# DanielLin94144/E2E-ASR-Pytorch

Hardware: AMD Instinct MI355X
Metric: audio frames/sec (fwd+bwd) LibriSpeech-100 joint CTC-att (higher is better)
Workload: dtype bf16; 1 GPU; config/librispeech_asr.yaml (vgg 0, 4xBiLSTM-320, joint CTC-att 0.5), B=16 x T=1200 x D=160 per GPU, L=180, delta+SpecAugment on GPU, fwd+losses+bwd+grad-allreduce+clip+Adadelta, dropout on; global_batch=16, frames_per_utt=1200, parallelism=dp1

## Files before the change

e2e-asr-pytorch_amd/csrc/decoder_cluster.h:

```cpp
#pragma once
#include "common.h"
#include "handoff.h"
#include "decoder_internal.h"
#include <stdlib.h>
#include <algorithm>

namespace {


constexpr u64 PAIR_MASK = 7ull | (7ull << 32);
__device__ __forceinline__ u64 pair_want(unsigned seq, unsigned epoch) {
    epoch = 2u + epoch % 14u;
    const unsigned tag = ((epoch & 15u) << 2) | seq;
    return (u64)(tag & 7u) | ((u64)(tag >> 3) << 32);
}
__device__ __forceinline__ u64 pack2(float a, float b, u64 want) {
    return ((u64)(__float_as_uint(a) & ~7u) | ((u64)(__float_as_uint(b) & ~7u) << 32)) | want;
}
__device__ __forceinline__ float lo_f(u64 g) { return __uint_as_float((unsigned)g & ~7u); }
__device__ __forceinline__ float hi_f(u64 g) { return __uint_as_float((unsigned)(g >> 32) & ~7u); }
__device__ __forceinline__ unsigned f2h_bits(float x) { return (unsigned)__builtin_bit_cast(unsigned short, (_Float16)x); }
__device__ __forceinline__ u64 pack4h(float a, float b, float c, float d, u64 want) {
    const unsigned lo = (f2h_bits(a) & ~7u) | (f2h_bits(b) << 16), hi = (f2h_bits(c) & ~7u) | (f2h_bits(d) << 16);
    return ((u64)lo | ((u64)hi << 32)) | want;
// ... 35 lines not shown
__device__ __forceinline__ float tanh_f(float x) { return 1.f - 2.f * __builtin_amdgcn_rcpf(1.f + __expf(2.f * x)); }
__device__ __forceinline__ float sigm_f(float x) { return __builtin_amdgcn_rcpf(1.f + __expf(-x)); }

__device__ __forceinline__ float wave_sum_dpp(float v) {
#define DPB_STEP(CTRL, RMASK) v += __builtin_bit_cast(float, __builtin_amdgcn_update_dpp(0, __builtin_bit_cast(int, v), CTRL, RMASK, 0xf, false));
    DPB_STEP(0xB1, 0xf)
    DPB_STEP(0x4E, 0xf)
    DPB_STEP(0x141, 0xf)
    DPB_STEP(0x140, 0xf)
    DPB_STEP(0x142, 0xa)
    DPB_STEP(0x143, 0xc)
#undef DPB_STEP
    return __builtin_bit_cast(float, __builtin_amdgcn_readlane(__builtin_bit_cast(int, v), 63));
}
__device__ __forceinline__ float sum8_dpp(float v) {
    v += __builtin_bit_cast(float, __builtin_amdgcn_update_dpp(0, __builtin_bit_cast(int, v), 0xB1, 0xf, 0xf, false));
    v += __builtin_bit_cast(float, __builtin_amdgcn_update_dpp(0, __builtin_bit_cast(int, v), 0x4E, 0xf, 0xf, false));
    v += __builtin_bit_cast(float, __builtin_amdgcn_update_dpp(0, __builtin_bit_cast(int, v), 0x141, 0xf, 0xf, false));
    return v;
}
__device__ __forceinline__ float wave_max_dpp(float v) {
#define DPB_STEP(CTRL, RMASK) v = fmaxf(v, __builtin_bit_cast(float, __builtin_amdgcn_update_dpp(__builtin_bit_cast(int, v), __builtin_bit_cast(int, v), CTRL, RMASK, 0xf, false)));
    DPB_STEP(0xB1, 0xf)
    DPB_STEP(0x4E, 0xf)
    DPB_STEP(0x141, 0xf)
    DPB_STEP(0x140, 0xf)
    DPB_STEP(0x142, 0xa)
    DPB_STEP(0x143, 0xc)
#undef DPB_STEP
    return __builtin_bit_cast(float, __builtin_amdgcn_readlane(__builtin_bit_cast(int, v), 63));
}

struct PD {
    asr_dec_dims_t d;
    asr_dec_weights_t w;
    asr_dec_state_t s;
    const float* enc;
    const int64_t* enc_len;
    const unsigned short* wcat16;
    const float* embproj;
    u64* xbuf;
    unsigned* status;
    int NT, TE, UPW, QPW, CPW;
    int HG2, QG2, SG2;
    int KC, KCP;
    int allow_local;
    unsigned epoch;
};

struct ConvGeo { int NKS, WKP, IMG_LD, need; };
__host__ __device__ inline ConvGeo conv_geo(int TEB, int Ks) {
    ConvGeo g;
    g.NKS = (2 * Ks + 1 + 31) >> 5;
    g.WKP = 32 * g.NKS + 8;
    g.need = ((TEB + 15) & ~15) + 32 * g.NKS + 8;
    g.IMG_LD = ((g.need - 32 + 127) / 128) * 128 + 32;
    return g;
}
__host__ __device__ inline int conv_img_shorts(const ConvGeo& g) { return 8 * g.IMG_LD + 32 * g.WKP; }

struct FCarve { int cvx_shorts, img, shorts, WT, ATP, NG, x2, q, wg, attp, wc, epart, e, w, g, cpart, stage, stage_floats, floats; };
__host__ __device__ inline FCarve fwd_carve(int TEB, int NT, int A, int E, int Kn, int Ks, int KCP, int UPW, int SG2) {
    FCarve c;
    c.cvx_shorts = TEB * FCVX_LD;
    c.img = (c.cvx_shorts + 7) & ~7;
    c.shorts = (c.img + conv_img_shorts(conv_geo(TEB, Ks)) + 7) & ~7;
    c.WT = (2 * Ks + 1 + 3) & ~3;
    c.ATP = (NT * TEB + 2 * Ks + 8 + 3) & ~3;
    const int nch = E >> 3;
    c.NG = (64 * NCW) / nch; if (c.NG > 8) c.NG = 8;
    int o = 0;
    c.x2 = o; o += 2 * KCP;
    c.q = o; o += (A + 3) & ~3;
    c.wg = o; o += (A + 3) & ~3;
    c.attp = o; o += c.ATP;
    c.wc = o;
    c.epart = o; o += NCW * TEB;
    c.e = o; o += TEB;
    c.w = o; o += TEB;
    c.g = o; o += (4 * UPW + 3) & ~3;
    c.cpart = o; o += c.NG * E;
    c.stage = o;
    c.stage_floats = NT * 2 * SG2; if (c.stage_floats < Kn * TEB) c.stage_floats = Kn * TEB;
    o += c.stage_floats;
    c.floats = o;
    return c;
}

__device__ inline void conv_build_wimg(const float* __restrict__ Wconv, int Kn, int taps, const ConvGeo& g, unsigned short* wimg, int tid, int nthr) {
    for (int i = tid; i < 16 * g.WKP; i += nthr) {
        const int n = i / g.WKP, x = i - n * g.WKP;
        const float v = (n < Kn && x < taps) ? Wconv[n * taps + x] : 0.f;
        const __bf16 hi = (__bf16)v, lo = (__bf16)(v - (float)hi);
        wimg[i] = __builtin_bit_cast(unsigned short, hi);
        wimg[16 * g.WKP + i] = __builtin_bit_cast(unsigned short, lo);
    }
}

__device__ inline void conv_build_ximg(const float* src, int navail, const ConvGeo& g, unsigned short* ximg, int tz, int nthr) {
    const int ngrp = g.IMG_LD >> 2;
    for (int it = tz; it < 4 * ngrp; it += nthr) {
        const int c = it / ngrp, gq = it - c * ngrp;
        unsigned short h[4], l[4];
#pragma unroll
        for (int e = 0; e < 4; ++e) {
            const int i = 4 * gq + c + e;
            const float v = (i < navail && i < g.need) ? src[i] : 0.f;
            const __bf16 hi = (__bf16)v, lo = (__bf16)(v - (float)hi);
            h[e] = __builtin_bit_cast(unsigned short, hi); l[e] = __builtin_bit_cast(unsigned short, lo);
        }
        *reinterpret_cast<uint2*>(ximg + (long)c * g.IMG_LD + 4 * gq) = make_uint2((unsigned)h[0] | ((unsigned)h[1] << 16), (unsigned)h[2] | ((unsigned)h[3] << 16));
        *reinterpret_cast<uint2*>(ximg + (long)(4 + c) * g.IMG_LD + 4 * gq) = make_uint2((unsigned)l[0] | ((unsigned)l[1] << 16), (unsigned)l[2] | ((unsigned)l[3] << 16));
    }
}

template <int NW, class Epi>
__device__ inline void conv_mfma(const unsigned short* ximg, const unsigned short* wimg, const ConvGeo& g, int MTB, int wave, int lane, Epi epi) {
    constexpr int CT = 3;
    const int m = lane & 15, q = lane >> 4, cc = m & 3;
    const unsigned short* xh = ximg + (long)cc * g.IMG_LD + (m - cc) + 8 * q;
    const unsigned short* xl = xh + 4 * g.IMG_LD;
    const unsigned short* wh = wimg + m * g.WKP + 8 * q;
    const unsigned short* wl = wh + 16 * g.WKP;
    for (int mt0 = wave; mt0 < MTB; mt0 += NW * CT) {
        f32x4 acc[CT];
#pragma unroll
        for (int c = 0; c < CT; ++c) acc[c] = f32x4{0.f, 0.f, 0.f, 0.f};
        for (int ks = 0; ks < g.NKS; ++ks) {
            const bf16x8 bh = *reinterpret_cast<const bf16x8*>(wh + 32 * ks), bl = *reinterpret_cast<const bf16x8*>(wl + 32 * ks);
#pragma unroll
            for (int c = 0; c < CT; ++c) {
                const int mt = mt0 + NW * c;
                if (mt < MTB) {
                    const unsigned short* ph = xh + 16 * mt + 32 * ks;
                    const unsigned short* pl = xl + 16 * mt + 32 * ks;
                    const uint2 h0 = *reinterpret_cast<const uint2*>(ph), h1 = *reinterpret_cast<const uint2*>(ph + 4);
                    const uint2 l0 = *reinterpret_cast<const uint2*>(pl), l1 = *reinterpret_cast<const uint2*>(pl + 4);
                    const bf16x8 ah = __builtin_bit_cast(bf16x8, make_uint4(h0.x, h0.y, h1.x, h1.y));
                    const bf16x8 al = __builtin_bit_cast(bf16x8, make_uint4(l0.x, l0.y, l1.x, l1.y));
                    acc[c] = mma16(bh, ah, acc[c]);
                    acc[c] = mma16(bl, ah, acc[c]);
                    acc[c] = mma16(bh, al, acc[c]);
                }
            }
        }
#pragma unroll
        for (int c = 0; c < CT; ++c) {
            const int mt = mt0 + NW * c;
            if (mt < MTB) epi(mt, m, q, acc[c]);
        }
    }
}

__device__ __forceinline__ void compute_barrier(unsigned* cnt, unsigned& gen) {
    gen += NCW;
    __builtin_amdgcn_fence(__ATOMIC_RELEASE, "workgroup");
    if ((threadIdx.x & 63) == 0) {
        __hip_atomic_fetch_add(cnt, 1u, __ATOMIC_RELAXED, __HIP_MEMORY_SCOPE_WORKGROUP);
        while (__hip_atomic_load(cnt, __ATOMIC_RELAXED, __HIP_MEMORY_SCOPE_WORKGROUP) < gen) __builtin_amdgcn_s_sleep(1);
    }
    __builtin_amdgcn_fence(__ATOMIC_ACQUIRE, "workgroup");
}

__global__ void build_wcat16_kernel(const float* __restrict__ wih, const float* __restrict__ whh, unsigned short* __restrict__ out,
                                    int rows, int Dd, int E, int KCP) {
    const long total = (long)rows * KCP;
    for (long i = blockIdx.x * (long)blockDim.x + threadIdx.x; i < total; i += (long)gridDim.x * blockDim.x) {
        const int r = (int)(i / KCP), k = (int)(i - (long)r * KCP);
        float v = 0.f;
        if (k < E) v = wih[(long)r * (Dd + E) + Dd + k];
        else if (k < E + Dd) v = whh[(long)r * Dd + (k - E)];
        out[i] = f2bf_bits(v);
    }
}

template <typename K>
bool grid_resident(K kernel, int grid, int block, size_t lds) {
    int per_cu = 0;
    if (hipOccupancyMaxActiveBlocksPerMultiprocessor(&per_cu, kernel, block, lds) != hipSuccess || per_cu < 1) return false;
    int dev = 0, cus = 0;
    if (hipGetDevice(&dev) != hipSuccess || hipDeviceGetAttribute(&cus, hipDeviceAttributeMultiprocessorCount, dev) != hipSuccess) return false;
    return grid <= cus;
}

template <int CH>
__device__ __forceinline__ void poll_copy(const u64* src, int n16, float* dst, int gt, int np, u64 want, unsigned* status) {
    for (int i0 = gt; i0 < n16; i0 += CH * np) {
        u64 lo[CH], hi[CH];
        int cnt = 0;
#pragma unroll
        for (int k = 0; k < CH; ++k) if (i0 + k * np < n16) cnt = k + 1;
        gather16<CH>(src + 2 * i0, 2 * np, cnt, PAIR_MASK, want, lo, hi, status);
#pragma unroll
        for (int k = 0; k < CH; ++k)
            if (k < cnt) *reinterpret_cast<float4*>(dst + 4 * (long)(i0 + k * np)) = make_float4(lo_f(lo[k]), hi_f(lo[k]), lo_f(hi[k]), hi_f(hi[k]));
    }
}

constexpr int EPOCH_WORD = 1008;
constexpr size_t STATUS_CLEAR_BYTES = 4032;
__global__ void bump_epoch_kernel(unsigned* status) { status[EPOCH_WORD] = status[EPOCH_WORD] + 1u; }
__global__ void clear_work_kernel(uint4* work, long n16) {
    for (long i = blockIdx.x * (long)blockDim.x + threadIdx.x; i < n16; i += (long)gridDim.x * blockDim.x)
        if (i < (long)(STATUS_CLEAR_BYTES / 16) || i >= 256) work[i] = make_uint4(0u, 0u, 0u, 0u);
}
inline void clear_work(void* work, size_t xbuf_bytes, hipStream_t st) {
    const long n16 = (long)((4096 + xbuf_bytes) / 16);
    hipLaunchKernelGGL(clear_work_kernel, dim3((unsigned)std::min<long>((n16 + 255) / 256, 2048)), dim3(256), 0, st, (uint4*)work, n16);
}

}
```

e2e-asr-pytorch_amd/csrc/decoder_persist.hip:

```cpp
#include "decoder_plan.h"

static int g_persist_fwd = -1, g_persist_bwd = -1;
static int g_stream_fwd = -1, g_stream_bwd = -1;
extern "C" int asr_att_decoder_set_persistent(int flags) {
    const int old = (g_persist_fwd != 0 ? 1 : 0) | (g_persist_bwd != 0 ? 2 : 0) | (g_stream_fwd > 0 ? 4 : 0) | (g_stream_bwd > 0 ? 8 : 0);
    g_persist_fwd = flags & 1; g_persist_bwd = (flags >> 1) & 1; g_stream_fwd = (flags >> 2) & 1; g_stream_bwd = (flags >> 3) & 1;
    return old;
}
static void read_switches() {
    if (g_persist_fwd < 0) g_persist_fwd = env_switch("ASR_DEC_PERSIST", 1);
    if (g_persist_bwd < 0) g_persist_bwd = env_switch("ASR_DEC_PERSIST_BWD", 1);
    if (g_stream_fwd < 0) g_stream_fwd = env_switch("ASR_DEC_STREAM", 0);
    if (g_stream_bwd < 0) g_stream_bwd = env_switch("ASR_DEC_STREAM", 0);
}
static FwdPlan fwd_plan(const asr_dec_dims_t& d) { read_switches(); return chosen_plan(persist_plan(d), stream_plan_f(d), g_stream_fwd); }
static BwdPlan bwd_plan(const asr_dec_dims_t& d) { read_switches(); return chosen_plan(persist_plan_b(d), stream_plan_b(d), g_stream_bwd); }

DecPlanInfo dec_fwd_plan_info(const asr_dec_dims_t& d) {
    read_switches();
    const FwdPlan r = persist_plan(d), s = stream_plan_f(d);
    return {chosen_plan(r, s, g_stream_fwd).kind, 0, 0, std::max(r.total, s.total)};
}
DecPlanInfo dec_bwd_plan_info(const asr_dec_dims_t& d) {
    read_switches();
    const BwdPlan r = persist_plan_b(d), s = stream_plan_b(d), pl = chosen_plan(r, s, g_stream_bwd);
    return {pl.kind, pl.NT, std::max(r.NT, s.NT), std::max(r.total, s.total)};
}
float* dec_bwd_dgates(const asr_dec_dims_t& d, void* work) { return bwd_work(d, bwd_plan(d), work).dgates; }

namespace {

size_t dec_fwd_persist_lds(int TE, int NT, int A, int E, int Ks, int KCP, int UPW, int SG2) {
    const int EPL = 16 * cdiv(TE, 16);
    const ConvGeo cg = conv_geo(EPL, Ks);
    const size_t shorts = (size_t)((TE * A + 7) & ~7)
                        + ((TE * E + 7) & ~7)
                        + EPL * FCVX_LD
                        + 8 * cg.IMG_LD
                        + 32 * cg.WKP;
    const size_t floats = (size_t)2 * KCP
                        + ((A + 3) & ~3)
                        + ((A + 3) & ~3)
                        + ((NT * TE + 2 * Ks + 8 + 3) & ~3)
                        + NCW * EPL
                        + ((4 * UPW + 3) & ~3)
                        + (size_t)NT * 2 * SG2;
    return 2 * shorts + 4 * floats;
}

template <int KNMAX, int TPW>
__global__ __launch_bounds__(64 * (NCW + NPW)) void dec_fwd_persist(PD p) {
    constexpr int TE = 8 * TPW;
    constexpr int MT = (TE + 15) / 16;
    constexpr int EPL = 16 * MT;
    extern __shared__ __attribute__((aligned(16))) unsigned char smem[];
    __shared__ unsigned s_bar;
    __shared__ float s_scale[NCW][32];
    const asr_dec_dims_t& d = p.d;
    const int id = blockIdx.x, xcd = id & 7, slot = id >> 3;
    const int cb = slot / p.NT, j = slot - cb * p.NT;
    const int b = cb * 8 + xcd;
    if (b >= d.B) return;
    const unsigned epoch_ = __builtin_amdgcn_readfirstlane(p.status[EPOCH_WORD]);
    const int tid = threadIdx.x, lane = tid & 63, wave = __builtin_amdgcn_readfirstlane(tid >> 6);
    const int NT = p.NT, A = d.A, E = d.E, Dd = d.Dd, Tp = d.Tp, Kn = d.Kn, Ks = d.Ks, L = d.L;
    const int taps = 2 * Ks + 1, XW = Dd + E;
    const int tau0 = j * TE;
    const int len = min((int)p.enc_len[b], Tp);
    const int tmax = max(len - 1, 0);
    unsigned short* s_key = reinterpret_cast<unsigned short*>(smem);
    unsigned short* s_enc = s_key + ((TE * A + 7) & ~7);
    unsigned short* s_cvx = s_enc + ((TE * E + 7) & ~7);
    const ConvGeo cg_ = conv_geo(EPL, Ks);
    unsigned short* s_ximg = s_cvx + EPL * FCVX_LD;
    unsigned short* s_wimg = s_ximg + 8 * cg_.IMG_LD;
    float* s_x2 = reinterpret_cast<float*>(s_wimg + 32 * cg_.WKP);
    float* s_q = s_x2 + 2 * p.KCP;
    float* s_wg = s_q + ((A + 3) & ~3);
    const int WT = (taps + 3) & ~3;
    const int ATP = (NT * TE + 2 * Ks + 8 + 3) & ~3;
    float* s_attp = s_wg + ((A + 3) & ~3);
    float* s_epart = s_attp + ATP;
    float* s_g = s_epart + NCW * EPL;
    float* s_stage = s_g + ((4 * p.UPW + 3) & ~3);
    if (tid == 0) s_bar = 0u;
    const long region = (long)NT * (p.HG2 + p.QG2 + p.SG2);
    auto xb = [&](int parity) { return p.xbuf + ((long)parity * d.B + b) * region; };
    for (int parity = 0; parity < 2; ++parity) {
        u64* base = xb(parity);
        for (int i = tid; i < p.HG2; i += blockDim.x) st_gran_local(base + (long)j * p.HG2 + i, 0ull);
        for (int i = tid; i < p.QG2; i += blockDim.x) st_gran_local(base + (long)NT * p.HG2 + (long)j * p.QG2 + i, 0ull);
        for (int i = tid; i < p.SG2; i += blockDim.x) st_gran_local(base + (long)NT * (p.HG2 + p.QG2) + (long)j * p.SG2 + i, 0ull);
    }
    asm volatile("s_waitcnt vmcnt(0)" ::: "memory");
    __syncthreads();
    const bool local = xcd_consensus(reinterpret_cast<u64*>(p.status) + 64 + b, NT, p.allow_local, p.status);

    for (int i = tid; i < TE * A; i += blockDim.x) {
        const int f = i / A, a = i - f * A;
        s_key[((long)(f >> 2) * A + a) * 4 + (f & 3)] = f2bf_bits(p.s.key[((long)b * Tp + min(tau0 + f, tmax)) * A + a]);
    }
    for (int i = tid; i < TE * E; i += blockDim.x) {
        const int f = i / E, c = i - f * E;
        s_enc[i] = f2bf_bits(p.enc[((long)b * Tp + min(tau0 + f, tmax)) * E + c]);
    }
    for (int i = tid; i < EPL * FCVX_LD; i += blockDim.x) s_cvx[i] = 0;
    conv_build_wimg(p.w.Wconv, Kn, taps, cg_, s_wimg, tid, blockDim.x);
    for (int i = tid; i < A; i += blockDim.x) s_wg[i] = p.w.wg[i];
    for (int i = tid; i < 2 * p.KCP; i += blockDim.x) s_x2[i] = 0.f;
    {
        const float uni = 1.f / (float)max(len, 1);
        for (int i = tid; i < ATP; i += blockDim.x) {
            const int tau = i - Ks;
            s_attp[i] = (tau >= 0 && tau < len) ? uni : 0.f;
        }
    }
    __syncthreads();

    if (wave >= NCW) {
        const int gt = tid - 64 * NCW, np = 64 * NPW;
        for (int t = 0; t < L; ++t) {
            if (t > 0) {
                const u64* src = xb((t - 1) & 1);
                const u64 want = pair_want(seq_of(t - 1), epoch_);
                for (int i0 = gt; 2 * i0 < NT * p.HG2; i0 += np) {
                    u64 lo[1], hi[1];
                    gather16<1>(src + 2 * i0, 0, 1, PAIR_MASK, want, lo, hi, p.status);
                    const int g0 = 2 * i0, prod = g0 / p.HG2, gi = g0 - prod * p.HG2;
                    const int u = prod * p.UPW + 2 * gi;
                    const float v[4] = {lo_f(lo[0]), hi_f(lo[0]), lo_f(hi[0]), hi_f(hi[0])};
#pragma unroll
                    for (int k = 0; k < 4; ++k)
                        if (2 * gi + k < p.UPW && u + k < Dd) s_x2[(t & 1) * p.KCP + E + u + k] = v[k];
                }
            }
            DP_JIT(0)
            __syncthreads();
            DP_JIT(1)
            {
                const u64* src = xb(t & 1) + (long)NT * p.HG2;
                const u64 want = pair_want(seq_of(t), epoch_);
                for (int i0 = gt; 2 * i0 < NT * p.QG2; i0 += np) {
                    u64 lo[1], hi[1];
                    gather16<1>(src + 2 * i0, 0, 1, PAIR_MASK, want, lo, hi, p.status);
                    const int g0 = 2 * i0, prod = g0 / p.QG2, gi = g0 - prod * p.QG2;
                    const int a = prod * p.QPW + 2 * gi;
                    const float v[4] = {lo_f(lo[0]), hi_f(lo[0]), lo_f(hi[0]), hi_f(hi[0])};
#pragma unroll
                    for (int k = 0; k < 4; ++k)
                        if (2 * gi + k < p.QPW && a + k < A) s_q[a + k] = v[k];
                }
            }
            DP_JIT(2)
            __syncthreads();
            DP_JIT(3)
            {
                const u64* src = xb(t & 1) + (long)NT * (p.HG2 + p.QG2);
                const u64 want = pair_want(seq_of(t), epoch_);
                const int npair = NT * p.SG2 / 2;
                for (int i0 = gt; i0 < npair; i0 += 10 * np) {
                    u64 lo[10], hi[10];
                    int cnt = 0;
#pragma unroll
                    for (int k = 0; k < 10; ++k) if (i0 + k * np < npair) cnt = k + 1;
                    gather16<10>(src + 2 * i0, 2 * np, cnt, PAIR_MASK, want, lo, hi, p.status);
#pragma unroll
                    for (int k = 0; k < 10; ++k)
                        if (k < cnt) {
                            float4* o = reinterpret_cast<float4*>(s_stage + 4 * (long)(i0 + k * np));
                            *o = make_float4(lo_f(lo[k]), hi_f(lo[k]), lo_f(hi[k]), hi_f(hi[k]));
                        }
                }
            }
            DP_JIT(4)
            __syncthreads();
            DP_JIT(5)
        }
        return;
    }

    unsigned gen = 0;
    const int u_base = j * p.UPW, q_base = j * p.QPW, c_base = j * p.CPW;
    const int SG2f = 2 * p.SG2;
    const float bg = p.w.bg[0];
    float c_state = 0.f;
    const int RPW = (4 * p.UPW + NCW - 1) / NCW;
    const int nu_cnt = (((A + 15) >> 4) - wave + NCW - 1) / NCW;
    bf16x8 wpx[FSW_NU];
    float wgu[FSW_NU];
    {
        const int q = lane >> 4, c = lane & 15;
#pragma unroll
        for (int nu = 0; nu < FSW_NU; ++nu) {
            const int a = 16 * (wave + NCW * nu) + c;
            const bool ok = a < A;
            const float* wr = p.w.Wproj + (long)min(a, A - 1) * Kn;
#pragma unroll
            for (int i = 0; i < 8; ++i) {
                const int slot = 8 * q + i;
                const int k = slot < KNMAX ? slot : (slot < 2 * KNMAX ? slot - KNMAX : slot - 2 * KNMAX);
                const float w = (ok && slot < 3 * KNMAX && k < Kn) ? wr[min(k, Kn - 1)] : 0.f;
                const __bf16 hi = (__bf16)w;
                wpx[nu][i] = (slot < 2 * KNMAX) ? hi : (__bf16)(w - (float)hi);
            }
            wgu[nu] = ok ? p.w.wg[min(a, A - 1)] : 0.f;
        }
    }
    constexpr int QR = 2;
    float wq0[QR][5], wq1[QR][5], bq0[QR], bq1[QR];
#pragma unroll
    for (int r2 = 0; r2 < QR; ++r2) {
        const int o0 = 2 * wave + 2 * NCW * r2;
        const int a0 = min(q_base + o0, A - 1), a1 = min(q_base + o0 + 1, A - 1);
        bq0[r2] = p.w.bq[a0]; bq1[r2] = p.w.bq[a1];
#pragma unroll
        for (int k = 0; k < 5; ++k) {
            const int kk = min(lane + 64 * k, Dd - 1);
            wq0[r2][k] = p.w.Wq[(long)a0 * Dd + kk];
            wq1[r2][k] = p.w.Wq[(long)a1 * Dd + kk];
        }
    }
    DP_DECL

    for (int t = 0; t < L; ++t) {
        int tz = tid, lz_ = lane;
        asm volatile("" : "+v"(tz), "+v"(lz_));
        const int lane = lz_;
        const long row = (long)b * L + t;
        float* s_x = s_x2 + (t & 1) * p.KCP;
        const u64 want = pair_want(seq_of(t), epoch_);
        u64* out = xb(t & 1);
        float add_r = 0.f;
        {
            const int r = wave * RPW + lane;
            if (lane < RPW && r < 4 * p.UPW) {
                const int g = r / p.UPW, ul = r - g * p.UPW, unit = u_base + ul;
                if (unit < Dd) {
                    const int grow = g * Dd + unit;
                    add_r = p.embproj[row * 4 * Dd + grow] + p.w.bih[0][grow] + p.w.bhh[0][grow];
                }
            }
        }
        DP_MARK(0)
        __syncthreads();
        DP_MARK(1)
        for (int o0 = 2 * wave, rd = 0; o0 < p.QPW; o0 += 2 * NCW, ++rd) {
            float acc0 = 0.f, acc1 = 0.f;
            const int a0 = min(q_base + o0, A - 1), a1 = min(q_base + o0 + 1, A - 1);
            float b0 = 0.f, b1 = 0.f;
            if (rd < QR) {
#pragma unroll
                for (int r2 = 0; r2 < QR; ++r2) if (r2 == rd) { b0 = bq0[r2]; b1 = bq1[r2]; }
            } else {
                b0 = p.w.bq[a0]; b1 = p.w.bq[a1];
            }
            if (t > 0) {
                float w0[5], w1[5];
                if (rd < QR) {
#pragma unroll
                    for (int r2 = 0; r2 < QR; ++r2)
                        if (r2 == rd) {
#pragma unroll
                            for (int k = 0; k < 5; ++k) { w0[k] = wq0[r2][k]; w1[k] = wq1[r2][k]; }
                        }
                } else {
#pragma unroll
                    for (int k = 0; k < 5; ++k) {
                        const int kk = min(lane + 64 * k, Dd - 1);
                        w0[k] = p.w.Wq[(long)a0 * Dd + kk];
                        w1[k] = p.w.Wq[(long)a1 * Dd + kk];
                    }
                }
#pragma unroll
                for (int k = 0; k < 5; ++k) {
                    const float hv = (lane + 64 * k < Dd) ? s_x[E + lane + 64 * k] : 0.f;
                    acc0 += w0[k] * hv; acc1 += w1[k] * hv;
                }
                for (int kk = lane + 320; kk < Dd; kk += 64) { const float hv = s_x[E + kk]; acc0 += p.w.Wq[(long)a0 * Dd + kk] * hv; acc1 += p.w.Wq[(long)a1 * Dd + kk] * hv; }
                acc0 = wave_sum_dpp(acc0); acc1 = wave_sum_dpp(acc1);
            }
            if (lane == 0) {
                const float q0 = tanh_f(acc0 + b0), q1 = tanh_f(acc1 + b1);
                u64* dst = out + (long)NT * p.HG2 + (long)j * p.QG2 + (o0 >> 1);
                if (local) publish<true>(dst, pack2(q0, q1, want)); else publish<false>(dst, pack2(q0, q1, want));
                if (q_base + o0 < A) p.s.q[row * A + q_base + o0] = q0;
                if (o0 + 1 < p.QPW && q_base + o0 + 1 < A) p.s.q[row * A + q_base + o0 + 1] = q1;
            }
        }
        if (tz == 0 && (p.QPW + 1) / 2 < p.QG2) {
            u64* dst = out + (long)NT * p.HG2 + (long)j * p.QG2 + p.QG2 - 1;
            if (local) publish<true>(dst, pack2(0.f, 0.f, want)); else publish<false>(dst, pack2(0.f, 0.f, want));
        }
        DP_MARK(2)
        {
            conv_build_ximg(s_attp + tau0, ATP - tau0, cg_, s_ximg, tz, 64 * NCW);
            compute_barrier(&s_bar, gen);
            conv_mfma<NCW>(s_ximg, s_wimg, cg_, MT, wave, lane, [&](int mt, int n, int q4, const f32x4& acc) {
                const int i = 16 * mt + n;
                unsigned short* r = s_cvx + i * FCVX_LD;
#pragma unroll
                for (int pp = 0; pp < 2; ++pp) {
                    const int k0 = 4 * q4 + 2 * pp;
                    if (k0 < Kn && i < TE) {
                        const float v0 = acc[2 * pp], v1 = acc[2 * pp + 1];
                        const __bf16 h0 = (__bf16)v0, h1 = (__bf16)v1;
                        const __bf16 l0 = (__bf16)(v0 - (float)h0), l1 = (__bf16)(v1 - (float)h1);
                        const unsigned hh = (unsigned)__builtin_bit_cast(unsigned short, h0) | ((unsigned)__builtin_bit_cast(unsigned short, h1) << 16);
                        const unsigned ll = (unsigned)__builtin_bit_cast(unsigned short, l0) | ((unsigned)__builtin_bit_cast(unsigned short, l1) << 16);
                        *reinterpret_cast<unsigned*>(r + k0) = hh;
                        *reinterpret_cast<unsigned*>(r + KNMAX + k0) = ll;
                        *reinterpret_cast<unsigned*>(r + 2 * KNMAX + k0) = hh;
                        if (p.s.conv && tau0 + i < Tp) {
                            p.s.conv[(row * Kn + k0) * Tp + tau0 + i] = v0;
                            if (k0 + 1 < Kn) p.s.conv[(row * Kn + k0 + 1) * Tp + tau0 + i] = v1;
                        }
                    }
                }
            });
        }
        DP_MARK(3)
        __syncthreads();
        DP_MARK(4)
        {
            int opaque = 0;
            asm volatile("" : "+v"(opaque));
            const int q = (lane >> 4) + opaque, c = lane & 15;
            float ep[MT][4];
#pragma unroll
            for (int mt = 0; mt < MT; ++mt)
#pragma unroll
                for (int r = 0; r < 4; ++r) ep[mt][r] = 0.f;
            float qv[FSW_NU];
#pragma unroll
            for (int nu = 0; nu < FSW_NU; ++nu) qv[nu] = s_q[min(16 * (wave + NCW * nu) + c, A - 1)];
#pragma unroll
            for (int mt = 0; mt < MT; ++mt) {
                const int f0 = 16 * mt + 4 * q;
                const bf16x8 av = *reinterpret_cast<const bf16x8*>(s_cvx + (16 * mt + c) * FCVX_LD + 8 * q);
                const int fg = min(f0, TE - 4) >> 2;
#pragma unroll
                for (int nu = 0; nu < FSW_NU; ++nu) {
                    if (nu < nu_cnt) {
                        const int a = min(16 * (wave + NCW * nu) + c, A - 1);
                        const f32x4 lp = mma16(av, wpx[nu], f32x4{0.f, 0.f, 0.f, 0.f});
                        const uint2 kb = *reinterpret_cast<const uint2*>(s_key + ((long)fg * A + a) * 4);
                        const float key[4] = {__uint_as_float(kb.x << 16), __uint_as_float(kb.x & 0xffff0000u),
                                              __uint_as_float(kb.y << 16), __uint_as_float(kb.y & 0xffff0000u)};
#pragma unroll
                        for (int r = 0; r < 4; ++r) ep[mt][r] += wgu[nu] * tanh_f(key[r] + qv[nu] + tanh_f(lp[r]));
                    }
                }
            }
#pragma unroll
            for (int mt = 0; mt < MT; ++mt)
#pragma unroll
                for (int r = 0; r < 4; ++r) {
                    float v = ep[mt][r];
#define DPF_STEP(CTRL) v += __builtin_bit_cast(float, __builtin_amdgcn_update_dpp(0, __builtin_bit_cast(int, v), CTRL, 0xf, 0xf, false));
                    DPF_STEP(0xB1) DPF_STEP(0x4E) DPF_STEP(0x141) DPF_STEP(0x140)
#undef DPF_STEP
                    if (c == 0) s_epart[wave * EPL + 16 * mt + 4 * q + r] = v;
                }
        }
        DP_MARK(5)
        compute_barrier(&s_bar, gen);
        DP_MARK(6)
        {
            float ev = NEG_BIG;
            if (lane < TE) {
                float sv = 0.f;
#pragma unroll
                for (int w8 = 0; w8 < NCW; ++w8) sv += s_epart[w8 * EPL + lane];
                if (tau0 + lane < len) ev = (sv + bg) / d.temperature;
            }
            const float m = wave_max_dpp(ev);
            const float wv = (ev > 0.5f * NEG_BIG) ? __expf(ev - m) : 0.f;
            const float ssum = wave_sum_dpp(wv);
            const int c2 = tz;
            float x0 = 0.f, x1 = 0.f;
            if (2 * c2 < E) {
#pragma unroll
                for (int f = 0; f < TE; ++f) {
                    const float wf = __builtin_bit_cast(float, __builtin_amdgcn_readlane(__builtin_bit_cast(int, wv), f));
                    const unsigned pr = *reinterpret_cast<const unsigned*>(s_enc + f * E + 2 * c2);
                    x0 += wf * __uint_as_float(pr << 16);
                    x1 += wf * __uint_as_float(pr & 0xffff0000u);
                }
            }
            u64* rec = out + (long)NT * (p.HG2 + p.QG2) + (long)j * p.SG2;
            const int ghead = (TE + 2) >> 1;
            const float y0 = __shfl_down(x0, 1), y1 = __shfl_down(x1, 1);
            if (2 * c2 < E && (c2 & 1) == 0) {
                if (local) publish<true>(rec + ghead + (c2 >> 1), pack4h(x0, x1, y0, y1, want)); else publish<false>(rec + ghead + (c2 >> 1), pack4h(x0, x1, y0, y1, want));
            }
            if (wave == NCW - 1) {
                const float e0 = __shfl(ev, min(2 * lane, 63)), e1 = __shfl(ev, min(2 * lane + 1, 63));
                if (lane < TE / 2) {
                    if (local) publish<true>(rec + lane, pack2(e0, e1, want)); else publish<false>(rec + lane, pack2(e0, e1, want));
                } else if (lane == TE / 2) {
                    if (local) publish<true>(rec + lane, pack2(m, ssum, want)); else publish<false>(rec + lane, pack2(m, ssum, want));
                } else if (lane == TE / 2 + 1 && ghead + E / 4 < p.SG2) {
                    u64* dst = rec + p.SG2 - 1;
                    if (local) publish<true>(dst, pack2(0.f, 0.f, want)); else publish<false>(dst, pack2(0.f, 0.f, want));
                }
            }
        }
        DP_MARK(7)
        __syncthreads();
        DP_MARK(8)
        {
            float mi = NEG_BIG, si = 0.f;
            if (lane < NT) { mi = s_stage[lane * SG2f + TE]; si = s_stage[lane * SG2f + TE + 1]; }
            const float M = wave_max_dpp(mi);
            const float wi = (lane < NT) ? si * __expf(mi - M) : 0.f;
            const float S = fmaxf(wave_sum_dpp(wi), 1e-30f);
            const float invS = 1.f / S;
            if (lane < 32) s_scale[wave][lane] = (lane < NT) ? __expf(mi - M) * invS : 0.f;
            __builtin_amdgcn_fence(__ATOMIC_RELEASE, "workgroup");
            __builtin_amdgcn_fence(__ATOMIC_ACQUIRE, "workgroup");
            for (int tau = tz; tau < Tp; tau += 64 * NCW) {
                const int i = tau / TE, f = tau - i * TE;
                const float ev = s_stage[i * SG2f + f];
                const float av = (ev > 0.5f * NEG_BIG) ? __expf(ev - M) * invS : 0.f;
                s_attp[Ks + tau] = av;
                if (i == j) p.s.att[row * Tp + tau] = av;
            }
            for (int c2_ = tz; 2 * c2_ < E; c2_ += 64 * NCW) {
                float a0 = 0.f, a1 = 0.f;
                for (int i = 0; i < NT; ++i) {
                    const unsigned w_ = __float_as_uint(s_stage[i * SG2f + TE + 2 + c2_]);
                    a0 += h2f_lo(w_) * s_scale[wave][i]; a1 += h2f_hi(w_) * s_scale[wave][i];
                }
                const int c = 2 * c2_;
                s_x[c] = a0; s_x[c + 1] = a1;
                if (c >= c_base && c < c_base + p.CPW) p.s.xin[row * XW + Dd + c] = a0;
                if (c + 1 >= c_base && c + 1 < c_base + p.CPW) p.s.xin[row * XW + Dd + c + 1] = a1;
            }
        }
        DP_MARK(9)
        compute_barrier(&s_bar, gen);
        DP_MARK(10)
        {
            constexpr int RBF = 10;
            const int nchunk = p.KCP >> 3;
            float mine = 0.f;
#pragma unroll 1
            for (int bt = 0; bt * RBF < RPW; ++bt) {
                float part[RBF];
#pragma unroll
                for (int rr = 0; rr < RBF; ++rr) part[rr] = 0.f;
                for (int ch0 = lane; ch0 < nchunk; ch0 += 128) {
                    uint4 wv[RBF][2];
#pragma unroll
                    for (int rr = 0; rr < RBF; ++rr) {
                        const int r = min(wave * RPW + bt * RBF + rr, 4 * p.UPW - 1);
                        const int g = r / p.UPW, ul = r - g * p.UPW;
                        const long grow = (long)g * Dd + min(u_base + ul, Dd - 1);
#pragma unroll
                        for (int h2 = 0; h2 < 2; ++h2)
                            wv[rr][h2] = *reinterpret_cast<const uint4*>(p.wcat16 + grow * p.KCP + 8 * min(ch0 + 64 * h2, nchunk - 1));
                    }
#pragma unroll
                    for (int h2 = 0; h2 < 2; ++h2) {
                        const int ch = ch0 + 64 * h2;
                        if (ch < nchunk) {
                            const float4 xa = *reinterpret_cast<const float4*>(s_x + 8 * ch);
                            const float4 xb4 = *reinterpret_cast<const float4*>(s_x + 8 * ch + 4);
#pragma unroll
                            for (int rr = 0; rr < RBF; ++rr) {
                                const uint4 w4 = wv[rr][h2];
                                part[rr] += __uint_as_float(w4.x << 16) * xa.x + __uint_as_float(w4.x & 0xffff0000u) * xa.y +
                                            __uint_as_float(w4.y << 16) * xa.z + __uint_as_float(w4.y & 0xffff0000u) * xa.w +
                                            __uint_as_float(w4.z << 16) * xb4.x + __uint_as_float(w4.z & 0xffff0000u) * xb4.y +
                                            __uint_as_float(w4.w << 16) * xb4.z + __uint_as_float(w4.w & 0xffff0000u) * xb4.w;
                            }
                        }
                    }
                }
#pragma unroll
                for (int rr = 0; rr < RBF; ++rr) {
                    const float sv = wave_sum_dpp(part[rr]);
                    if (lane == bt * RBF + rr) mine = sv;
                }
            }
            const int r = wave * RPW + lane;
            if (lane < RPW && r < 4 * p.UPW) s_g[r] = mine + add_r;
        }
        DP_MARK(11)
        compute_barrier(&s_bar, gen);
        DP_MARK(12)
        if (wave == 0) {
            const int unit = u_base + lane;
            const bool uok = lane < p.UPW && unit < Dd;
            float hv = 0.f;
            float ai = 0.f, af = 0.f, ag = 0.f, ao = 0.f;
            if (uok) {
                ai = sigm_f(s_g[lane]); af = sigm_f(s_g[p.UPW + lane]);
                ag = tanh_f(s_g[2 * p.UPW + lane]); ao = sigm_f(s_g[3 * p.UPW + lane]);
                c_state = af * c_state + ai * ag;
                hv = ao * tanh_f(c_state);
            }
            const float hn = __shfl_down(hv, 1);
            if (t + 1 < L && (lane & 1) == 0 && lane < 2 * p.HG2) {
                u64* dst = out + (long)j * p.HG2 + (lane >> 1);
                if (local) publish<true>(dst, pack2(hv, hn, want)); else publish<false>(dst, pack2(hv, hn, want));
            }
            if (uok) {
                float* go = p.s.gates + row * 4 * Dd;
                go[unit] = ai; go[Dd + unit] = af; go[2 * Dd + unit] = ag; go[3 * Dd + unit] = ao;
                p.s.cs[row * Dd + unit] = c_state;
                p.s.hs[row * Dd + unit] = hv;
            }
        }
        DP_MARK(13)
    }
    DP_DUMP
}

FwdPlan persist_plan(const asr_dec_dims_t& d) {
    if (d.NL != 1 || d.B > 64 || d.A > 16 * FSW_NU * NCW || d.Kn > 10 || (d.E & 7) != 0 || d.Dd > 20 * 32 || d.Tp < 1) return FwdPlan{};
    const int cpx = cdiv(d.B, 8);
    const int cand[] = {2, 4, 5, 8};
    FwdPlan pl{};
    for (int i = 0; i < 4 && !pl.tpw; ++i) {
        const int nt = cdiv(d.Tp, 8 * cand[i]);
        if (nt <= 30 && cpx * nt <= 32) pl.tpw = cand[i];
    }
    if (!pl.tpw) return FwdPlan{};
    pl.kind = 1; pl.TE = 8 * pl.tpw; pl.NT = cdiv(d.Tp, pl.TE);
    fwd_sizes(d, pl);
    if (pl.UPW > 64 || cdiv(4 * pl.UPW, NCW) > 60) return FwdPlan{};
    pl.lds = dec_fwd_persist_lds(pl.TE, pl.NT, d.A, d.E, d.Ks, pl.KCP, pl.UPW, pl.SG2);
    if (getenv("ASR_DEC_PLAN_DEBUG")) fprintf(stderr, "[asr] resident fwd plan B=%d T'=%d: NT=%d TE=%d UPW=%d LDS=%zu\n", d.B, d.Tp, pl.NT, pl.TE, pl.UPW, pl.lds);
    return pl.lds > 156 * 1024 ? FwdPlan{} : pl;
}

}

int dec_fwd_persistent(const asr_dec_dims_t& d, const asr_dec_weights_t& w, const asr_dec_state_t& s, const float* enc,
                       const int64_t* enc_len, void* work, size_t work_bytes, hipStream_t st) {
    read_switches();
    if (!g_persist_fwd) return 1;
    const FwdPlan pl = fwd_plan(d);
    if (pl.kind == 2) return dec_fwd_streamed(d, w, s, enc, enc_len, work, work_bytes, st);
    if (!pl.kind || !work || work_bytes < pl.total || ((uintptr_t)work & 255) != 0 || !s.conv) return 1;
    const FwdWork wk = fwd_work(d, pl, work);
    clear_work(work, wk.xbuf_bytes, st);
    hipLaunchKernelGGL(build_wcat16_kernel, dim3(512), dim3(256), 0, st, w.Wih[0], w.Whh[0], wk.wcat16, 4 * d.Dd, d.Dd, d.E, pl.KCP);
    const int XW = d.Dd + d.E;
    int rc = asr_gemm(s.xin, w.Wih[0], wk.embproj, nullptr, d.B * d.L, 4 * d.Dd, d.Dd, XW, XW, 4 * d.Dd, 1, 1, ASR_ACT_NONE, 0, 1, 1, 0, 0, 0,
                      0, 0, ASR_BF16, (asr_stream_t)st);
    if (rc != ASR_OK) return rc;
    const PD p{d, w, s, enc, enc_len, wk.wcat16, wk.embproj, wk.xbuf, wk.status, pl.NT, pl.TE, pl.UPW, pl.QPW, pl.CPW, pl.HG2, pl.QG2, pl.SG2, pl.KC,
               pl.KCP, xcd_local_allowed()};
    const ClusterLaunch go{"asr_att_decoder_fwd(persistent)", 160 * 1024 - 2048, cluster_grid(d, pl.NT), dim3(64 * (NCW + NPW)), pl.lds, st};
    if (d.Kn <= 4) {
        if (pl.tpw == 2) return go.run<dec_fwd_persist<4, 2>>(p);
        if (pl.tpw == 4) return go.run<dec_fwd_persist<4, 4>>(p);
        if (pl.tpw == 5) return go.run<dec_fwd_persist<4, 5>>(p);
        return go.run<dec_fwd_persist<4, 8>>(p);
    }
    if (pl.tpw == 2) return go.run<dec_fwd_persist<10, 2>>(p);
    if (pl.tpw == 4) return go.run<dec_fwd_persist<10, 4>>(p);
    if (pl.tpw == 5) return go.run<dec_fwd_persist<10, 5>>(p);
    return 1;
}

namespace {

template <int KNMAX, int TEC>
__global__ __launch_bounds__(512) void dec_bwd_persist(PB p) {
    extern __shared__ __attribute__((aligned(16))) unsigned char smem[];
    __shared__ unsigned s_bar;
    __shared__ float s_red[8];
    constexpr int KP = (KNMAX + 3) & ~3;
    const int TE = TEC ? TEC : p.TE;
    const int MT = (TE + 15) / 16;
    const asr_dec_dims_t& d = p.d;
    const int id = blockIdx.x, xcd = id & 7, slot_id = id >> 3;
    const int cb = slot_id / p.NT, j = slot_id - cb * p.NT;
    const int b = cb * 8 + xcd;
    if (b >= d.B) return;
    const unsigned epoch_ = __builtin_amdgcn_readfirstlane(p.status[EPOCH_WORD]);
    const int tid = threadIdx.x, lane = tid & 63, wave = __builtin_amdgcn_readfirstlane(tid >> 6);
    const int NT = p.NT, A = d.A, E = d.E, Dd = d.Dd, Tp = d.Tp, Kn = d.Kn, Ks = d.Ks, L = d.L;
    const int ncw = (A + 63) >> 6, nct = 64 * ncw, nw = ncw + NPB;
    const int taps = 2 * Ks + 1, XW = Dd + E, R4 = p.R4;
    const int tau0 = j * TE;
    const int len = min((int)p.enc_len[b], Tp);
    const int tmax = max(len - 1, 0);
    const BCarve cv_ = bwd_carve(TE, KP, A, E, Kn, Ks, NT, p.UPW, p.CG2, p.QG2, p.NG2);
    const int AP = cv_.AP, DW = cv_.DW, PADL = cv_.PADL, WT = cv_.WT, AQ = cv_.AQ;
    const int TW = NT * TE;
    const int CG2f = 2 * p.CG2, NG2f = 2 * p.NG2, QG2f = 2 * p.QG2;
    unsigned short* s_sh = reinterpret_cast<unsigned short*>(smem);
    unsigned short* s_key = s_sh + cv_.key;
    unsigned short* s_dl = s_sh + cv_.dl;
    unsigned short* s_wp16 = s_sh + cv_.wp16;
    unsigned short* s_dg16 = s_sh + cv_.dg16;
    unsigned short* s_wq16 = s_sh + cv_.wq16;
    unsigned short* s_cvx = s_sh + cv_.cvx;
    unsigned short* s_cvT = s_sh + cv_.cvT;
    float* s_f = reinterpret_cast<float*>(s_sh + cv_.shorts);
    float* s_wc = s_f + cv_.wc;
    float* s_crec = s_f + cv_.crec;
    float* s_qst = s_f + cv_.qst;
    float* s_nrec = s_f + cv_.nrec;
    float* s_dcp = s_f + cv_.dcp;
    float* s_de = s_f + cv_.de;
    float* s_out = s_f + cv_.out;
    float* s_hq = s_f + cv_.hq;
    float* s_pt = s_f + cv_.pt;
    float* s_dcx = s_f + cv_.dcx;
    float* s_dq = s_f + cv_.dq;
    const long region = (long)NT * (p.CG2 + p.QG2 + p.VG2 + p.NG2);
    auto xb = [&](int parity) { return p.xbuf + ((long)parity * d.B + b) * region; };
    const long offC = 0, offQ = offC + (long)NT * p.CG2, offV = offQ + (long)NT * p.QG2, offN = offV + (long)NT * p.VG2;
    if (tid == 0) s_bar = 0u;
    for (int parity = 0; parity < 2; ++parity) {
        u64* base = xb(parity);
        for (int i = tid; i < p.CG2; i += blockDim.x) st_gran_local(base + offC + (long)j * p.CG2 + i, 0ull);
        for (int i = tid; i < p.QG2; i += blockDim.x) st_gran_local(base + offQ + (long)j * p.QG2 + i, 0ull);
        for (int i = tid; i < p.VG2; i += blockDim.x) st_gran_local(base + offV + (long)j * p.VG2 + i, 0ull);
        for (int i = tid; i < p.NG2; i += blockDim.x) st_gran_local(base + offN + (long)j * p.NG2 + i, 0ull);
    }
    asm volatile("s_waitcnt vmcnt(0)" ::: "memory");
    __syncthreads();
    const bool local = xcd_consensus(reinterpret_cast<u64*>(p.status) + 64 + b, NT, p.allow_local, p.status);

    for (int i = tid; i < TE * A; i += blockDim.x) {
        const int f = i / A, a = i - f * A;
        s_key[((long)(f >> 2) * A + a) * 4 + (f & 3)] = f2bf_bits(p.s.key[((long)b * Tp + min(tau0 + f, tmax)) * A + a]);
    }
    for (int i = tid; i < 16 * AP; i += blockDim.x) { const int k = i / AP, a = i - k * AP; s_wp16[i] = (k < Kn && a < A) ? f2bf_bits(p.w.Wproj[a * Kn + k]) : (unsigned short)0; }
    for (int i = tid; i < Kn * WT; i += blockDim.x) { const int k = i / WT, jj = i - k * WT; s_wc[i] = (jj < taps) ? p.w.Wconv[k * taps + jj] : 0.f; }
    for (int i = tid; i < 64 * KCHB * 4; i += blockDim.x) s_dg16[i] = 0;
    for (int i = tid; i < NT * NG2f + 8; i += blockDim.x) s_nrec[i] = 0.f;
    for (int i = tid; i < NT * CG2f; i += blockDim.x) s_crec[i] = 0.f;
    for (int i = tid; i < Kn * DW; i += blockDim.x) s_dcp[i] = 0.f;
    for (int i = tid; i < TE * AP; i += blockDim.x) s_dl[i] = 0;
    for (int i = tid; i < 16 * SW_MT * CVX_LD; i += blockDim.x) s_cvx[i] = 0;
    for (int i = tid; i < 16 * CVT_LD; i += blockDim.x) s_cvT[i] = 0;
    for (int i = tid; i < 16 * SW_MT; i += blockDim.x) s_de[i] = 0.f;
    const int u_base = j * p.UPW, c_base = j * p.CPW;
    for (int i = tid; i < p.UPW * AQ; i += blockDim.x) {
        const int ul = i / AQ, aa = i - ul * AQ;
        s_wq16[i] = (aa < A && u_base + ul < Dd) ? f2bf_bits(p.wqT[(long)(u_base + ul) * A + aa]) : (unsigned short)0;
    }
    const int nout = p.CPW + p.UPW;
    const int nunits = (A + 15) >> 4;
    const int nu_cnt = (nunits - wave + nw - 1) / nw;
    const int qsub = lane >> 4, csub = lane & 15;
    __syncthreads();

    if (wave >= ncw) {
        const int gt = tid - nct, np = 64 * NPB;
        const int vp0 = max(0, (tau0 - Ks) / TE), vp1 = min(NT - 1, (tau0 + TE - 1 + Ks) / TE);
        const int obase = RCB * ncw + (wave - ncw);
        uint2 wreg[RPB][KCHB];
        DPB_WLOAD(RPB, obase, NPB)
        Sweep<SW_NUP> S;
        sweep_init<KNMAX>(S, p.w.Wproj, p.w.wg, A, Kn, wave, nw, lane);
        for (int t = L - 1; t >= 0; --t) {
            const int s = L - 1 - t;
            const u64 want = pair_want(seq_of(s), epoch_);
            const u64* base = xb(s & 1);
            DP_JIT(6)
            __syncthreads();
            DPB_P1(RPB, obase, NPB)
            __syncthreads();
            poll_copy<4>(base + offC, NT * p.CG2 / 2, s_crec, gt, np, want, p.status);
            float qa[SW_NUP];
#pragma unroll
            for (int nu = 0; nu < SW_NUP; ++nu) qa[nu] = p.s.q[((long)b * L + t) * A + min(16 * (wave + nw * nu) + csub, A - 1)];
            DP_JIT(7)
            __syncthreads();
            DP_JIT(8)
            __syncthreads();
            DPB_SWEEP_AND_PUBLISH(const_cast<u64*>(base), SW_NUP)
            __syncthreads();
            for (int z = 0; z < p.poll_delay; ++z) __builtin_amdgcn_s_sleep(127);
            {
                const int nq = NT * p.QG2 / 2, nv = (vp1 - vp0 + 1) * (p.VG2 / 2);
                const u64* vbase = base + offV + (long)vp0 * p.VG2;
                for (int i0 = gt; i0 < nq + nv; i0 += 10 * np) {
// ... 312 lines not shown
```

Baseline: 1.135 million frames/s.

## Move location-aware conv into producer waves, overlapping it with compute waves

```diff
diff --git a/e2e-asr-pytorch_amd/csrc/decoder_cluster.h b/e2e-asr-pytorch_amd/csrc/decoder_cluster.h
--- a/e2e-asr-pytorch_amd/csrc/decoder_cluster.h
+++ b/e2e-asr-pytorch_amd/csrc/decoder_cluster.h
@@ -211,13 +211,20 @@
     }
 }
 
-__device__ __forceinline__ void compute_barrier(unsigned* cnt, unsigned& gen) {
-    gen += NCW;
+template <int NW>
+__device__ __forceinline__ void wave_group_barrier(unsigned* cnt, unsigned& gen) {
+    gen += NW;
     __builtin_amdgcn_fence(__ATOMIC_RELEASE, "workgroup");
     if ((threadIdx.x & 63) == 0) {
         __hip_atomic_fetch_add(cnt, 1u, __ATOMIC_RELAXED, __HIP_MEMORY_SCOPE_WORKGROUP);
         while (__hip_atomic_load(cnt, __ATOMIC_RELAXED, __HIP_MEMORY_SCOPE_WORKGROUP) < gen) __builtin_amdgcn_s_sleep(1);
     }
+    __builtin_amdgcn_fence(__ATOMIC_ACQUIRE, "workgroup");
+}
+__device__ __forceinline__ void compute_barrier(unsigned* cnt, unsigned& gen) { wave_group_barrier<NCW>(cnt, gen); }
+__device__ __forceinline__ void barrier_reached(unsigned* cnt, unsigned target) {
+    if ((threadIdx.x & 63) == 0)
+        while (__hip_atomic_load(cnt, __ATOMIC_RELAXED, __HIP_MEMORY_SCOPE_WORKGROUP) < target) __builtin_amdgcn_s_sleep(1);
     __builtin_amdgcn_fence(__ATOMIC_ACQUIRE, "workgroup");
 }
 
diff --git a/e2e-asr-pytorch_amd/csrc/decoder_persist.hip b/e2e-asr-pytorch_amd/csrc/decoder_persist.hip
--- a/e2e-asr-pytorch_amd/csrc/decoder_persist.hip
+++ b/e2e-asr-pytorch_amd/csrc/decoder_persist.hip
@@ -30,7 +30,7 @@
 
 namespace {
 
-size_t dec_fwd_persist_lds(int TE, int NT, int A, int E, int Ks, int KCP, int UPW, int SG2) {
+size_t dec_fwd_persist_lds(int TE, int NT, int A, int E, int Kn, int Ks, int KCP, int UPW, int SG2) {
     const int EPL = 16 * cdiv(TE, 16);
     const ConvGeo cg = conv_geo(EPL, Ks);
     const size_t shorts = (size_t)((TE * A + 7) & ~7)
@@ -44,7 +44,7 @@
                         + ((NT * TE + 2 * Ks + 8 + 3) & ~3)
                         + NCW * EPL
                         + ((4 * UPW + 3) & ~3)
-                        + (size_t)NT * 2 * SG2;
+                        + std::max(NT * 2 * SG2, Kn * EPL);
     return 2 * shorts + 4 * floats;
 }
 
@@ -54,7 +54,7 @@
     constexpr int MT = (TE + 15) / 16;
     constexpr int EPL = 16 * MT;
     extern __shared__ __attribute__((aligned(16))) unsigned char smem[];
-    __shared__ unsigned s_bar;
+    __shared__ unsigned s_bar, s_pbar;
     __shared__ float s_scale[NCW][32];
     const asr_dec_dims_t& d = p.d;
     const int id = blockIdx.x, xcd = id & 7, slot = id >> 3;
@@ -83,7 +83,8 @@
     float* s_epart = s_attp + ATP;
     float* s_g = s_epart + NCW * EPL;
     float* s_stage = s_g + ((4 * p.UPW + 3) & ~3);
-    if (tid == 0) s_bar = 0u;
+    float* s_cst = s_stage;
+    if (tid == 0) { s_bar = 0u; s_pbar = 0u; }
     const long region = (long)NT * (p.HG2 + p.QG2 + p.SG2);
     auto xb = [&](int parity) { return p.xbuf + ((long)parity * d.B + b) * region; };
     for (int parity = 0; parity < 2; ++parity) {
@@ -119,6 +120,32 @@
 
     if (wave >= NCW) {
         const int gt = tid - 64 * NCW, np = 64 * NPW;
+        unsigned pgen = 0;
+        auto conv_tile = [&]() {
+            conv_build_ximg(s_attp + tau0, ATP - tau0, cg_, s_ximg, gt, np);
+            wave_group_barrier<NPW>(&s_pbar, pgen);
+            conv_mfma<NPW>(s_ximg, s_wimg, cg_, MT, wave - NCW, lane, [&](int mt, int n, int q4, const f32x4& acc) {
+                const int i = 16 * mt + n;
+                unsigned short* r = s_cvx + i * FCVX_LD;
+#pragma unroll
+                for (int pp = 0; pp < 2; ++pp) {
+                    const int k0 = 4 * q4 + 2 * pp;
+                    if (k0 < Kn && i < TE) {
+                        const float v0 = acc[2 * pp], v1 = acc[2 * pp + 1];
+                        const __bf16 h0 = (__bf16)v0, h1 = (__bf16)v1;
+                        const __bf16 l0 = (__bf16)(v0 - (float)h0), l1 = (__bf16)(v1 - (float)h1);
+                        const unsigned hh = (unsigned)__builtin_bit_cast(unsigned short, h0) | ((unsigned)__builtin_bit_cast(unsigned short, h1) << 16);
+                        const unsigned ll = (unsigned)__builtin_bit_cast(unsigned short, l0) | ((unsigned)__builtin_bit_cast(unsigned short, l1) << 16);
+                        *reinterpret_cast<unsigned*>(r + k0) = hh;
+                        *reinterpret_cast<unsigned*>(r + KNMAX + k0) = ll;
+                        *reinterpret_cast<unsigned*>(r + 2 * KNMAX + k0) = hh;
+                        s_cst[k0 * EPL + i] = v0;
+                        if (k0 + 1 < Kn) s_cst[(k0 + 1) * EPL + i] = v1;
+                    }
+                }
+            });
+        };
+        conv_tile();
         for (int t = 0; t < L; ++t) {
             if (t > 0) {
                 const u64* src = xb((t - 1) & 1);
@@ -175,6 +202,11 @@
             DP_JIT(4)
             __syncthreads();
             DP_JIT(5)
+            if (t + 1 < L) {
+                barrier_reached(&s_bar, (unsigned)NCW * (3u * (unsigned)t + 2u));
+                DP_JIT(6)
+                conv_tile();
+            }
         }
         return;
     }
@@ -292,31 +324,9 @@
             if (local) publish<true>(dst, pack2(0.f, 0.f, want)); else publish<false>(dst, pack2(0.f, 0.f, want));
         }
         DP_MARK(2)
-        {
-            conv_build_ximg(s_attp + tau0, ATP - tau0, cg_, s_ximg, tz, 64 * NCW);
-            compute_barrier(&s_bar, gen);
-            conv_mfma<NCW>(s_ximg, s_wimg, cg_, MT, wave, lane, [&](int mt, int n, int q4, const f32x4& acc) {
-                const int i = 16 * mt + n;
-                unsigned short* r = s_cvx + i * FCVX_LD;
-#pragma unroll
-                for (int pp = 0; pp < 2; ++pp) {
-                    const int k0 = 4 * q4 + 2 * pp;
-                    if (k0 < Kn && i < TE) {
-                        const float v0 = acc[2 * pp], v1 = acc[2 * pp + 1];
-                        const __bf16 h0 = (__bf16)v0, h1 = (__bf16)v1;
-                        const __bf16 l0 = (__bf16)(v0 - (float)h0), l1 = (__bf16)(v1 - (float)h1);
-                        const unsigned hh = (unsigned)__builtin_bit_cast(unsigned short, h0) | ((unsigned)__builtin_bit_cast(unsigned short, h1) << 16);
-                        const unsigned ll = (unsigned)__builtin_bit_cast(unsigned short, l0) | ((unsigned)__builtin_bit_cast(unsigned short, l1) << 16);
-                        *reinterpret_cast<unsigned*>(r + k0) = hh;
-                        *reinterpret_cast<unsigned*>(r + KNMAX + k0) = ll;
-                        *reinterpret_cast<unsigned*>(r + 2 * KNMAX + k0) = hh;
-                        if (p.s.conv && tau0 + i < Tp) {
-                            p.s.conv[(row * Kn + k0) * Tp + tau0 + i] = v0;
-                            if (k0 + 1 < Kn) p.s.conv[(row * Kn + k0 + 1) * Tp + tau0 + i] = v1;
-                        }
-                    }
-                }
-            });
+        for (int idx = tz; idx < Kn * TE; idx += 64 * NCW) {
+            const int k = idx / TE, i = idx - k * TE;
+            if (p.s.conv && tau0 + i < Tp) p.s.conv[(row * Kn + k) * Tp + tau0 + i] = s_cst[k * EPL + i];
         }
         DP_MARK(3)
         __syncthreads();
@@ -530,7 +540,7 @@
     pl.kind = 1; pl.TE = 8 * pl.tpw; pl.NT = cdiv(d.Tp, pl.TE);
     fwd_sizes(d, pl);
     if (pl.UPW > 64 || cdiv(4 * pl.UPW, NCW) > 60) return FwdPlan{};
-    pl.lds = dec_fwd_persist_lds(pl.TE, pl.NT, d.A, d.E, d.Ks, pl.KCP, pl.UPW, pl.SG2);
+    pl.lds = dec_fwd_persist_lds(pl.TE, pl.NT, d.A, d.E, d.Kn, d.Ks, pl.KCP, pl.UPW, pl.SG2);
     if (getenv("ASR_DEC_PLAN_DEBUG")) fprintf(stderr, "[asr] resident fwd plan B=%d T'=%d: NT=%d TE=%d UPW=%d LDS=%zu\n", d.B, d.Tp, pl.NT, pl.TE, pl.UPW, pl.lds);
     return pl.lds > 156 * 1024 ? FwdPlan{} : pl;
 }
```

New measurement: 1.146 million frames/s (median of 6 runs). No clear change (+1.0%).
